# jackyko1991/vnet-tensorflow

Hardware: AMD Instinct MI355X
Metric: training patches/sec (128^3x1ch fp32) (higher is better)
Workload: dtype f32

## Files before the change

profiles/summarize.py:

```python
import csv
import json
import os
import shutil
import sys
from collections import defaultdict

LEGS = ("fp32", "x3", "c5", "c2")
KEEP = ("conv_kernel<", "wgrad_kernel<", "conv5_bf16", "wgrad5_bf16", "wgrad5_b16", "conv5_x3", "wgrad5_x3", "conv2_", "bn_", "input_")

FAMILIES = {
    "fp32": ("fp32", [("fwd", "conv_kernel<5, 1, 4, 8, 8, 4, 4, 1, false, 5, true", "2097152", 0),
                      ("bwd", "conv_kernel<5, 1, 4, 8, 8, 4, 4, 2, false, 5, false", "2097152", 0),
                      ("wgrad", "wgrad_kernel<5, 1, 4, 4, 16, 1, 16, 5", "131072", 0)]),
    "f32x3": ("x3", [("fwd", "conv5_x3_kernel<true, 1, false>", None, "longest"),
                     ("bwd", "conv5_x3_kernel<false, 2, false>", None, "longest"),
                     ("wgrad", "wgrad5_x3_kernel<false>", None, "longest")]),
    "bf16": ("c5", [("fwd", "conv5_bf16_c16pp_kernel<true>", None, "longest"),
                    ("bwd", "conv5_bf16_r32_kernel<false", None, 0),
                    ("wgrad", "wgrad5_bf16_rr_kernel<4, false>", None, 0)]),
}


def short(name):
    name = name.replace("(anonymous namespace)::", "").replace("void ", "")
    return name.split("(")[0]


def read_pass(path, counter):
    per_dispatch, meta = defaultdict(float), {}
    for r in csv.DictReader(open(path)):
        if r["Counter_Name"] != counter:
            continue
        key = int(r["Dispatch_Id"])
        per_dispatch[key] += float(r["Counter_Value"])
        meta[key] = (short(r["Kernel_Name"]), r["Grid_Size"], int(r["End_Timestamp"]) - int(r["Start_Timestamp"]))
    seqs = defaultdict(list)
    for key in sorted(per_dispatch):
        name, grid, dur = meta[key]
        seqs[(name, grid)].append((per_dispatch[key], dur))
    return seqs


def family_dispatches(src, here, tag):
    rows = []
    for fam, (leg, members) in FAMILIES.items():
        path = os.path.join(src, leg + "_kernel_trace.csv")
        if not os.path.exists(path):
            continue
        seqs, steps = defaultdict(list), 0
        trace = sorted(csv.DictReader(open(path)), key=lambda r: int(r["Start_Timestamp"]))
        for r in trace:
            name = short(r["Kernel_Name"])
            if name.startswith("softmax_dice_bwd_kernel"):
                steps += 1
            grid = r.get("Grid_Size") or str(int(r["Grid_Size_X"]) * int(r["Grid_Size_Y"]) * int(r["Grid_Size_Z"]))
            seqs[(name, grid)].append((int(r["Start_Timestamp"]), int(r["End_Timestamp"]) - int(r["Start_Timestamp"])))
        for role, pat, grid, pos in members:
            keys = [k for k in seqs if k[0].startswith(pat) and (grid is None or k[1] == grid)]
            if len(keys) != 1 or not steps:
                print("WARNING: %s/%s: %d kernels match" % (fam, role, len(keys)))
                continue
            seq = seqs[keys[0]]
            per_step = len(seq) // steps if len(seq) % steps == 0 else 1
            if pos == "longest":
                sel = [max(seq[i:i + per_step], key=lambda t: t[1]) for i in range(0, len(seq), per_step)]
            else:
                sel = seq[pos % per_step::per_step]
            for i, (t0, dur) in enumerate(sel):
                rows.append((fam, leg, role, keys[0][0], i, dur))
            d = sorted(t[1] for t in sel)
            print("%-6s %-6s %-40s n=%3d  avg %8.1f us  median %8.1f  min %8.1f  max %8.1f" %
                  (fam, role, keys[0][0][:40], len(d), sum(d) / len(d) / 1e3, d[len(d) // 2] / 1e3, d[0] / 1e3, d[-1] / 1e3))
    if rows:
        with open(os.path.join(here, tag + "_family_dispatches.csv"), "w") as f:
            f.write("family,leg,role,kernel,launch_index,duration_ns\n")
            for r in rows:
                f.write('%s,%s,%s,"%s",%d,%d\n' % r)


def main(src, tag):
    here = os.path.dirname(os.path.abspath(__file__))
    family_dispatches(src, here, tag)
    out = {"note": "per launch; KB from rocprofv3 --pmc (separate passes, one leg per run); fetch doubled per the gfx950 correction",
           "legs": {}, "families": {}}
    for leg in LEGS:
        st = os.path.join(src, leg + "_kernel_stats.csv")
        if os.path.exists(st):
            shutil.copy(st, os.path.join(here, "%s_kernel_stats_%s.csv" % (tag, leg)))
        seqs = {}
        for which, counter in (("fetch", "FETCH_SIZE"), ("write", "WRITE_SIZE")):
            path = os.path.join(src, "%s_%s_counter_collection.csv" % (leg, which))
            if os.path.exists(path):
                seqs[counter] = read_pass(path, counter)
        if not seqs:
            continue
        kern = {}
        for key in sorted(set().union(*[set(s) for s in seqs.values()])):
            name, grid = key
            if not name.startswith(KEEP):
# ... 63 lines not shown
```

vnet_tensorflow_amd/csrc/conv_kernels.h:

```cpp
#pragma once
#include "common.h"
#include <mutex>
#include <unordered_map>
#include <type_traits>
#include <vector>

namespace {

struct ConvArgs {
    const float* x0; const float* x1; int C0, C1, Cin;
    const float4* wp; const float* bias;
    float* y0; float* y1; int Cy0, Cy1, Cout;
    int B, Di, Hi, Wi, Do, Ho, Wo;
    int CQ;
    int CoutP;
    int nchunks, cps;
    int nbz, nby, nbx;
    int pad, padx;
    int vec_in, vec_out;
    float* part; size_t part_stride;
    int upO;
    int nz;
    int accum;
    const float* accsrc;
// ... 543 lines not shown
template <int KS, int STRIDE, int TZ, int TY, int TX, int NS, int TW, int KX = KS, bool IO16 = false>
__device__ __forceinline__ void wgrad_body(const WgradArgs& a, const int gid_x, const int gid_y, const int gid_z) {
#define VNET_WG_BID_X gid_x
#define VNET_WG_BID_Y gid_y
#define VNET_WG_BID_Z gid_z
#include "wgrad_body.inc"
#undef VNET_WG_BID_X
#undef VNET_WG_BID_Y
#undef VNET_WG_BID_Z
}

template <bool VEC>
__device__ __forceinline__ void wgrad_reduce_body(const float* __restrict__ part, int nsplit, int T3, int CinP, int CoutP,
                                                  int Cin, int Cout, float* __restrict__ dw, unsigned blk, unsigned nblk) {
    constexpr int W = VEC ? 4 : 1;
    __shared__ float sh[4][64 * W];
    const size_t total = (size_t)T3 * Cin * Cout / W;
    const size_t sstride = (size_t)T3 * CinP * CoutP;
    const int CoutG = Cout / W;
    const int o = threadIdx.x & 63, sg = threadIdx.x >> 6;
    for (size_t base = (size_t)blk * 64; base < total; base += (size_t)nblk * 64) {
        const size_t idx = base + o;
        float s[W];
#pragma unroll
        for (int j = 0; j < W; ++j) s[j] = 0.f;
        if (idx < total) {
            const int co = (int)(idx % CoutG) * W;
            const size_t r = idx / CoutG;
            const int ci = (int)(r % Cin), t = (int)(r / Cin);
            const float* p = part + ((size_t)t * CinP + ci) * CoutP + co;
            float acc[4][W];
#pragma unroll
            for (int u = 0; u < 4; ++u)
#pragma unroll
                for (int j = 0; j < W; ++j) acc[u][j] = 0.f;
            auto ld = [&](int k, float (&d)[W]) {
                if (VEC) { const float4 v = *reinterpret_cast<const float4*>(p + (size_t)k * sstride); d[0] += v.x; d[W > 1 ? 1 : 0] += v.y; d[W > 2 ? 2 : 0] += v.z; d[W > 3 ? 3 : 0] += v.w; }
                else d[0] += p[(size_t)k * sstride];
            };
            int k = sg;
            for (; k + 12 < nsplit; k += 16) { ld(k, acc[0]); ld(k + 4, acc[1]); ld(k + 8, acc[2]); ld(k + 12, acc[3]); }
            for (; k < nsplit; k += 4) ld(k, acc[0]);
#pragma unroll
            for (int j = 0; j < W; ++j) s[j] = (acc[0][j] + acc[1][j]) + (acc[2][j] + acc[3][j]);
        }
        __syncthreads();
#pragma unroll
        for (int j = 0; j < W; ++j) sh[sg][o * W + j] = s[j];
        __syncthreads();
        if (sg == 0 && idx < total) {
            float out[W];
#pragma unroll
            for (int j = 0; j < W; ++j) out[j] = sh[0][o * W + j] + sh[1][o * W + j] + sh[2][o * W + j] + sh[3][o * W + j];
            if (VEC) *reinterpret_cast<float4*>(dw + idx * 4) = make_float4(out[0], out[W > 1 ? 1 : 0], out[W > 2 ? 2 : 0], out[W > 3 ? 3 : 0]);
            else dw[idx] = out[0];
        }
    }
}

template <bool VEC>
__global__ void __launch_bounds__(256) wgrad_reduce_kernel(const float* __restrict__ part, int nsplit, int T3, int CinP, int CoutP,
                                                           int Cin, int Cout, float* __restrict__ dw) {
    wgrad_reduce_body<VEC>(part, nsplit, T3, CinP, CoutP, Cin, Cout, dw, blockIdx.x, gridDim.x);
}

}
namespace vnet_detail {
struct ReduceJob { const float* part; float* dw; int nsplit, T3, CinP, CoutP, Cin, Cout, vec; unsigned blk0; };
constexpr int REDUCE_BATCH = 32;
struct ReduceBatch { ReduceJob job[REDUCE_BATCH]; int n; };
struct DeferQueue { bool on = false; std::vector<ReduceJob> pending; };
struct DeferState { std::mutex mu; std::unordered_map<hipStream_t, DeferQueue> q; };
__attribute__((visibility("hidden"))) DeferState& defer_state();
struct Tuning {
    int wgrad_zs;
    int wgrad_rr;
    int conv_in4;
    double group_rounds;
    int group_debug;
    int bf16_deep;
    int bf16_deep_target;
    int bf16_c16pp;
    int x3_nb2;
    int f32_small;
};
__attribute__((visibility("hidden"))) Tuning& tuning();
}
namespace {
using vnet_detail::ReduceJob; using vnet_detail::ReduceBatch; using vnet_detail::REDUCE_BATCH;
using vnet_detail::DeferState; using vnet_detail::DeferQueue; using vnet_detail::defer_state; using vnet_detail::tuning;

__global__ void __launch_bounds__(256) wgrad_reduce_batched_kernel(ReduceBatch b) {
    int j = 0;
#pragma unroll 1
    for (int k = 1; k < b.n; ++k) if (blockIdx.x >= b.job[k].blk0) j = k;
    const ReduceJob& q = b.job[j];
    const unsigned nblk = (j + 1 < b.n ? b.job[j + 1].blk0 : gridDim.x) - q.blk0;
    if (q.vec) wgrad_reduce_body<true>(q.part, q.nsplit, q.T3, q.CinP, q.CoutP, q.Cin, q.Cout, q.dw, blockIdx.x - q.blk0, nblk);
    else wgrad_reduce_body<false>(q.part, q.nsplit, q.T3, q.CinP, q.CoutP, q.Cin, q.Cout, q.dw, blockIdx.x - q.blk0, nblk);
}


int launch_wgrad_reduce(const float* part, int nsplit, int T3, int CinP, int CoutP, int Cin, int Cout, float* dw, hipStream_t st) {
    const bool vec = (Cout % 4 == 0) && (CoutP % 4 == 0) && ((reinterpret_cast<uintptr_t>(dw) | reinterpret_cast<uintptr_t>(part)) & 15) == 0;
    {
        DeferState& ds = defer_state();
        std::lock_guard<std::mutex> lk(ds.mu);
        auto it = ds.q.find(st);
        if (it != ds.q.end() && it->second.on) {
            it->second.pending.push_back(ReduceJob{part, dw, nsplit, T3, CinP, CoutP, Cin, Cout, vec ? 1 : 0, 0u});
            return 0;
        }
    }
    const size_t total = (size_t)T3 * Cin * Cout / (vec ? 4 : 1);
    const int blocks = (int)min((size_t)4096, (total + 63) / 64);
    return with_bool(vec, [&](auto V) {
        return launch<wgrad_reduce_kernel<V>>(dim3(blocks), dim3(256), 0, st, part, nsplit, T3, CinP, CoutP, Cin, Cout, dw);
    });
}


__device__ __forceinline__ void pack_bf16_elem(int mode, const float* __restrict__ w, unsigned short* __restrict__ wp,
                                               int T, int I, int O, int ncob, size_t idx) {
    const int e = (int)(idx & 7);
    size_t q = idx >> 3;
    const int m = (int)(q & 31); q >>= 5;
    const int hf = (int)(q & 1); q >>= 1;
    const int cob = (int)(q % ncob); q /= ncob;
    const int t = (int)(q % T);
    const int chunk = (int)(q / T);
    const int k = chunk * 16 + hf * 8 + e, n = cob * 32 + m;
    float v = 0.f;
    if (mode == VNET_PACK_FWD_BF16) { if (k < I && n < O) v = w[((size_t)t * I + k) * O + n]; }
    else { if (k < O && n < I) v = w[((size_t)(T - 1 - t) * I + n) * O + k]; }
    wp[idx] = (unsigned short)(pk_bf16(v, 0.f) & 0xffffu);
}

#include "x3_pack.h"

__global__ void pack_kernel(int mode, const float* __restrict__ w, float* __restrict__ wp, int T, int I, int O,
                            int CQ, int NP, size_t total) {
    const bool r16 = (mode & VNET_PACK_ROUND_BF16) != 0;
    mode &= ~VNET_PACK_ROUND_BF16;
    for (size_t idx = (size_t)blockIdx.x * blockDim.x + threadIdx.x; idx < total; idx += (size_t)gridDim.x * blockDim.x) {
        const int r = (int)(idx & 3);
        size_t q = idx >> 2;
        const int n = (int)(q % NP); q /= NP;
        const int cq = (int)(q % CQ);
        const int t = (int)(q / CQ);
        const int k = cq * 4 + r;
        float v = 0.f;
        if (mode == VNET_PACK_FWD) {
            if (k < I && n < O) v = w[((size_t)t * I + k) * O + n];
        } else if (mode == VNET_PACK_BWD) {
            if (k < O && n < I) v = w[((size_t)(T - 1 - t) * I + n) * O + k];
        } else {
            if (k < I && n < 8 * O) v = w[(size_t)n * I + k];
        }
        wp[idx] = r16 ? bf_lo(pk_bf16(v, 0.f)) : v;
    }
}

#define VNET_PRIO_ALT(cond) do { if (cond) __builtin_amdgcn_s_setprio(1); else __builtin_amdgcn_s_setprio(0); } while (0)
#define VNET_PRIO_OFF() __builtin_amdgcn_s_setprio(0)

__global__ void __launch_bounds__(256) pack_batched_kernel(const long long* __restrict__ descs) {
// ... 1591 lines not shown
```

vnet_tensorflow_amd/csrc/conv_mfma.hip:

```cpp
#include "conv_kernels.h"
#include <string.h>

namespace vnet_detail {
DeferState& defer_state() { static DeferState s; return s; }
static Tuning tuning_from_env() {
    auto geti = [](const char* n, int d) { const char* e = getenv(n); return e ? atoi(e) : d; };
    Tuning t{};
    t.wgrad_zs = geti("VNET_WGRAD_ZS", 2); t.wgrad_rr = geti("VNET_WGRAD_RR", 1); t.conv_in4 = geti("VNET_CONV_IN4", 1);
    const char* g = getenv("VNET_WGRAD_GROUP_ROUNDS");
    t.group_rounds = g ? atof(g) : 2.0;
    t.group_debug = getenv("VNET_WGRAD_GROUP_DEBUG") ? 1 : 0;
    t.bf16_deep = geti("VNET_BF16_DEEP", 1); t.bf16_deep_target = geti("VNET_BF16_DEEP_TARGET", 256);
    t.f32_small = geti("VNET_F32_SMALL", 2); t.x3_nb2 = geti("VNET_X3_NB2", 1); t.bf16_c16pp = geti("VNET_BF16_C16PP", 1);
    return t;
}
Tuning& tuning() { static Tuning t = tuning_from_env(); return t; }
}

namespace {
double* option_slot(const char* name, int** ip) {
    vnet_detail::Tuning& t = vnet_detail::tuning();
    *ip = nullptr;
    if (!name) return nullptr;
    if (!strcmp(name, "WGRAD_ZS")) *ip = &t.wgrad_zs;
    else if (!strcmp(name, "WGRAD_RR")) *ip = &t.wgrad_rr;
    else if (!strcmp(name, "CONV_IN4")) *ip = &t.conv_in4;
    else if (!strcmp(name, "WGRAD_GROUP_DEBUG")) *ip = &t.group_debug;
    else if (!strcmp(name, "BF16_DEEP")) *ip = &t.bf16_deep;
    else if (!strcmp(name, "BF16_DEEP_TARGET")) *ip = &t.bf16_deep_target;
    else if (!strcmp(name, "F32_SMALL")) *ip = &t.f32_small;
    else if (!strcmp(name, "X3_NB2")) *ip = &t.x3_nb2;
    else if (!strcmp(name, "BF16_C16PP")) *ip = &t.bf16_c16pp;
    else if (!strcmp(name, "WGRAD_GROUP_ROUNDS")) return &t.group_rounds;
    return nullptr;
}
}

extern "C" {

double vnet_set_option(const char* name, double value) {
    int* ip; double* dp = option_slot(name, &ip);
    if (ip) { const double prev = *ip; *ip = (int)value; return prev; }
    if (dp) { const double prev = *dp; *dp = value; return prev; }
    return __builtin_nan("");
}
double vnet_get_option(const char* name) {
    int* ip; double* dp = option_slot(name, &ip);
    return ip ? (double)*ip : (dp ? *dp : __builtin_nan(""));
}

const char* vnet_version(void) { return "vnet_hip 0.2 (gfx950; fp32 MFMA 16x16x4, bf16 MFMA 32x32x16 / 16x16x32)"; }

size_t vnet_packed_weight_floats(int mode, int taps, int I, int O) {
    if (mode == VNET_PACK_FWD_X3 || mode == VNET_PACK_BWD_X3) {
        int nchunk, ncob; x3_packed_dims(mode == VNET_PACK_BWD_X3, I, O, &nchunk, &ncob);
        return (size_t)nchunk * X3_NPAIR * ncob * 3 * 256;
    }
    if (mode == VNET_PACK_FWD_BF16 || mode == VNET_PACK_BWD_BF16) {
        int nchunk, ncob; packed_dims_bf16(mode, I, O, &nchunk, &ncob);
        return (size_t)nchunk * taps * ncob * 512 / 2;
    }
    int Tp, CQ, NP; packed_dims(mode & ~VNET_PACK_ROUND_BF16, taps, I, O, &Tp, &CQ, &NP);
    return (size_t)Tp * CQ * NP * 4;
}

int vnet_pack_weights(int mode, const float* w, float* wp, int taps, int I, int O, void* stream) {
    if (!w || !wp || taps <= 0 || I <= 0 || O <= 0) return VNET_E_BADARG;
    if (mode == VNET_PACK_FWD_X3 || mode == VNET_PACK_BWD_X3) {
        if (taps != 125) return VNET_E_UNSUPPORTED;
        int nchunk, ncob; x3_packed_dims(mode == VNET_PACK_BWD_X3, I, O, &nchunk, &ncob);
        const uint32_t units = (uint32_t)nchunk * X3_NPAIR * ncob * 64;
        return launch<x3_pack_kernel>(dim3(min(4096u, (units + 255) / 256)), dim3(256), 0, (hipStream_t)stream,
                                      mode == VNET_PACK_BWD_X3 ? 1 : 0, w, reinterpret_cast<u32x4*>(wp), I, O, ncob, units);
    }
    if (mode == VNET_PACK_FWD_BF16 || mode == VNET_PACK_BWD_BF16) {
        int nchunk, ncob; packed_dims_bf16(mode, I, O, &nchunk, &ncob);
        const size_t total = (size_t)nchunk * taps * ncob * 512;
        const int blocks = (int)min((size_t)4096, (total + 255) / 256);
        return launch<pack_bf16_kernel>(dim3(blocks), dim3(256), 0, (hipStream_t)stream, mode, w,
                                        reinterpret_cast<unsigned short*>(wp), taps, I, O, ncob, total);
    }
    const int base = mode & ~VNET_PACK_ROUND_BF16;
    if (base < 0 || base > 2) return VNET_E_UNSUPPORTED;
    if (base == VNET_PACK_UP && taps != 8) return VNET_E_UNSUPPORTED;
    int Tp, CQ, NP; packed_dims(base, taps, I, O, &Tp, &CQ, &NP);
    const size_t total = (size_t)Tp * CQ * NP * 4;
    const int blocks = (int)min((size_t)4096, (total + 255) / 256);
    return launch<pack_kernel>(dim3(blocks), dim3(256), 0, (hipStream_t)stream, mode, w, wp, taps, I, O, CQ, NP, total);
}

int vnet_packed_dims(int mode, int taps, int I, int O, int* CQ, int* NP) {
    if (!CQ || !NP) return VNET_E_BADARG;
    if (mode == VNET_PACK_FWD_X3 || mode == VNET_PACK_BWD_X3) { x3_packed_dims(mode == VNET_PACK_BWD_X3, I, O, CQ, NP); return VNET_OK; }
    if (mode == VNET_PACK_FWD_BF16 || mode == VNET_PACK_BWD_BF16) { packed_dims_bf16(mode, I, O, CQ, NP); return VNET_OK; }
    mode &= ~VNET_PACK_ROUND_BF16;
    if (mode < 0 || mode > 2) return VNET_E_BADARG;
    int Tp; packed_dims(mode, taps, I, O, &Tp, CQ, NP);
    return VNET_OK;
}

int vnet_pack_weights_batched(const void* descs_dev, int n, void* stream) {
    if (!descs_dev || n <= 0) return VNET_E_BADARG;
    return launch<pack_batched_kernel>(dim3(512, n), dim3(256), 0, (hipStream_t)stream, (const long long*)descs_dev);
}

size_t vnet_conv_ws_bytes(int ks, int kx, int stride, int up, int Cin, int Cout, int B, int Do, int Ho, int Wo) {
    if (ks == 3 && (stride != 1 || up || (kx != 0 && kx != 3))) return 0;
    const int gridW = up ? (Wo + 1) / 2 : Wo;
    ConvPlan p = plan_conv(ks, stride, up, Cin, Cout, B, up ? (Do + 1) / 2 : Do, up ? (Ho + 1) / 2 : Ho, gridW, gridW);
    if (p.nsplit * p.nz <= 1) return 0;
    return (size_t)p.nsplit * p.nz * B * Do * Ho * Wo * round_up(Cout, 16) * sizeof(float);
}

int vnet_conv_stats_rows(int ks, int kx, int stride, int up, int Cin, int Cy0, int Cy1, int B, int Do, int Ho, int Wo) {
// ... 227 lines not shown
```

vnet_tensorflow_amd/csrc/conv_x3.h:

```cpp
#pragma once
#include "conv_kernels.h"

namespace {

constexpr int X3_TZ = 2, X3_TY = 8, X3_TX = 16;
constexpr int X3_IZ = X3_TZ + 4, X3_IY = X3_TY + 4, X3_IX = X3_TX + 4;
constexpr int X3_NV = X3_IZ * X3_IY * X3_IX;

template <bool W8>
struct X3G {
    static constexpr int TZ = W8 ? 4 : 2;
    static constexpr int IZ = TZ + 4, IY = X3_IY, IX = W8 ? 12 : X3_IX;
    static constexpr int ROWB = IX * 16;
    static constexpr int ZB = IY * ROWB + (W8 ? 64 : 0);
    static constexpr int PLANEB = IZ * ZB;
    static constexpr int PIECEB = 2 * PLANEB;
    static constexpr int TILEB = 3 * PIECEB;
    static constexpr int LDS = TILEB + 2 * 8 * 32 * 4;
    static constexpr int SPER = W8 ? 8 : 12;
};
static_assert(X3G<false>::PLANEB == X3_NV * 16 && X3G<false>::PLANEB % 256 == 0 && X3G<true>::PLANEB % 256 == 0, "tile planes");
static_assert((2 * X3G<true>::ZB) % 256 == 128, "lanes 8..15 of the narrow brick: the other half of the 256-byte bank row");
constexpr int X3_LDS = X3G<false>::LDS;

// ... 296 lines not shown
            const int oz = W8 ? bz * G::TZ + grp + 2 * (j >> 3) : bz * X3_TZ + grp, ox = W8 ? (j & 7) : bx * X3_TX + j;
            x3_for<2>([&](auto TI) {
                constexpr int t = decltype(TI)::value;
                const int oy = by * X3_TY + 2 * kw + t;
                if (oz < a.Do && oy < a.Ho && ox < a.Wo && co < a.Cout) {
                    const size_t ov = ((size_t)(b * a.Do + oz) * a.Ho + oy) * a.Wo + ox;
                    if (a.part) {
                        *reinterpret_cast<f32x4*>(a.part + (size_t)ks * a.part_stride + ov * a.CoutP + co) = o[t];
                        return;
                    }
                    float e[4] = {o[t][0] + bias4[0], o[t][1] + bias4[1], o[t][2] + bias4[2], o[t][3] + bias4[3]};
                    if constexpr (STATS) {
                        float4 rr = make_float4(0.f, 0.f, 0.f, 0.f);
                        if (a.res) rr = *reinterpret_cast<const float4*>(a.res + ov * a.Cout + co);
                        const float vv[4] = {e[0] + rr.x, e[1] + rr.y, e[2] + rr.z, e[3] + rr.w};
                        s1[0] += vv[0]; s1[1] += vv[1]; s1[2] += vv[2]; s1[3] += vv[3];
                        s2[0] += vv[0] * vv[0]; s2[1] += vv[1] * vv[1]; s2[2] += vv[2] * vv[2]; s2[3] += vv[3] * vv[3];
                    }
                    float* p = (co < a.Cy0) ? a.y0 + ov * a.Cy0 + co : a.y1 + ov * a.Cy1 + (co - a.Cy0);
                    if (a.accum) {
                        const float4 old = *reinterpret_cast<const float4*>(a.accsrc ? a.accsrc + ov * a.Cy0 + co : p);
                        e[0] += old.x; e[1] += old.y; e[2] += old.z; e[3] += old.w;
                    }
                    *reinterpret_cast<float4*>(p) = make_float4(e[0], e[1], e[2], e[3]);
                }
            });
            if constexpr (STATS) {
                x3_for<4>([&](auto KI) {
                    constexpr int k = decltype(KI)::value;
                    s1[k] = row16_sum(s1[k]); s2[k] = row16_sum(s2[k]);
                    if (j == 0) { sred[(nb * 8 + wave) * 32 + 4 * g + k] = s1[k]; sred[(nb * 8 + wave) * 32 + 16 + 4 * g + k] = s2[k]; }
                });
            }
            });
            __syncthreads();
            if constexpr (STATS) {
                int brick = (i_lo + slot + it * G8) / (ncobg * nks);
                x3_for<NB>([&](auto NBI) {
                    constexpr int nb = decltype(NBI)::value;
                    stats_row_write<8, 16>(sred + nb * 8 * 32, a.stats, (size_t)brick, (cob + nb) * 16, a.Cout, tid);
                });
            }
        }
        VNET_STAMP(6);
        if (last) zero_halo();
        if (more) tile_commit(((last ? 0 : lc + 1) & 1) ? 0x80000000u : 0u);
        VNET_STAMP(7);
        __syncthreads();
        VNET_STAMP(8);
        VNET_STAMP_FLUSH(step, wave, lane, 9);
    }
}

template <bool W8>
struct XWG {
    static constexpr int TZ = W8 ? 4 : 2;
    static constexpr int IZ = TZ + 4, IX = W8 ? 12 : X3_IX;
    static constexpr int XROW = IX * 32, XPLANE = X3_IY * XROW;
    static constexpr int XPB = IZ * XPLANE;
    static constexpr int DPB = 2 * X3_TY * 16 * 32;
    static constexpr int LDS = 3 * XPB + 3 * DPB;
    static constexpr int XHALF = W8 ? 2 * XPLANE : 8 * 32;
    static constexpr int XPER = W8 ? 8 : 12;
};
static_assert(XWG<false>::XROW % 256 == 128 && XWG<true>::XROW % 256 == 128, "row pairs of a k-step on disjoint banks");
constexpr int XW_LDS = XWG<false>::LDS;

__device__ __forceinline__ void xw_frag(bf16x8 (&F)[3], const unsigned char* lo, const unsigned char* hi, int pieceb) {
    typedef s16x4 __attribute__((address_space(3))) * lp;
#pragma unroll
    for (int s = 0; s < 3; ++s) {
        const s16x4 a = __builtin_amdgcn_ds_read_tr16_b64_v4i16((lp)(lo + s * pieceb));
        const s16x4 b = __builtin_amdgcn_ds_read_tr16_b64_v4i16((lp)(hi + s * pieceb));
        const s16x8 v = {a[0], a[1], a[2], a[3], b[0], b[1], b[2], b[3]};
        F[s] = __builtin_bit_cast(bf16x8, v);
    }
}

__device__ __forceinline__ void xw_mfma6(f32x4& acc, const bf16x8 (&A)[3], const bf16x8 (&B)[3]) {
#pragma unroll
    for (int k = 0; k < 6; ++k) acc = __builtin_amdgcn_mfma_f32_16x16x32_bf16(A[X3_PROD_A(k)], B[X3_PROD_B(k)], acc, 0, 0, 0);
}

template <bool W8>
__global__ void __launch_bounds__(512) __attribute__((amdgpu_waves_per_eu(2, 2))) wgrad5_x3_kernel(WgradArgs a) {
    constexpr int NT = 512;
    using G = XWG<W8>;
    constexpr int XW_XPB = G::XPB, XW_DPB = G::DPB, XW_XROW = G::XROW, XW_XPLANE = G::XPLANE;
    using XT = XTile<X3_IZ, X3_IY, X3_IX, NT>;
    static_assert(XT::PER == XWG<false>::XPER, "staging passes of the wide brick");
    extern __shared__ __attribute__((aligned(16))) unsigned char smem[];
    unsigned char* xt = smem;
    unsigned char* dyt = smem + 3 * XW_XPB;
    const int tid = threadIdx.x;
    const int lane = tid & 63, wave = __builtin_amdgcn_readfirstlane(tid >> 6);
    const int i = lane & 15, g = lane >> 4;
    const int split = blockIdx.x;
    const int chunk = blockIdx.y / a.ncob, cob = blockIdx.y - chunk * a.ncob;
    const int co0 = cob * 16;

    const int lane_x = W8 ? ((g & 1) * G::IX + (i >> 2)) * 32 + (g >> 1) * G::XHALF + (i & 3) * 8
                            : (((g & 1) * X3_IX + (g >> 1) * 8) + (i >> 2)) * 32 + (i & 3) * 8;
    const unsigned char* pb[3];
#pragma unroll
    for (int c = 0; c < 3; ++c) {
        const int q = 3 * wave + c, dz = q / 5, dx = q - dz * 5;
        pb[c] = xt + dz * XW_XPLANE + dx * 32 + lane_x;
    }
    const bool extra = wave < 5;
    const unsigned char* pe = xt + 4 * XW_XPLANE + (extra ? wave : 0) * XW_XROW + 4 * 32 + lane_x;
    const int lane_d = (((g & 1) * 16 + (g >> 1) * 8) + (i >> 2)) * 32 + (i & 3) * 8;
    const unsigned char* pa_lo = dyt + lane_d + (g & 1) * 128;
    const unsigned char* pa_hi = dyt + lane_d + (1 - (g & 1)) * 128;

    f32x4 acc[16];
#pragma unroll
    for (int t = 0; t < 16; ++t) acc[t] = f32x4{0.f, 0.f, 0.f, 0.f};

    float4 px[G::XPER], pd[2];
    auto brick_coords = [&](int brick, int& b, int& bz, int& by, int& bx) {
        bx = brick % a.nbx; brick /= a.nbx;
        by = brick % a.nby; brick /= a.nby;
        bz = brick % a.nbz; b = brick / a.nbz;
    };
    auto issue = [&](int brick) {
        int b, bz, by, bx;
        brick_coords(brick, b, bz, by, bx);
        if constexpr (W8) {
            const int stid = tid < 384 ? tid : tid - 128;
            const int iy = stid >> 5, col = stid & 31;
            const int c = chunk * 16 + (col & 3) * 4;
            const bool first = c < a.C0;
            const int cs = first ? a.C0 : a.C1;
            const float* src = (first ? a.x0 + c : a.x1 + (c - a.C0)) + (size_t)b * a.Di * a.Hi * a.Wi * cs;
            const int gz0 = bz * G::TZ - 2, gy = by * X3_TY - 2 + iy;
            const bool yok = (unsigned)gy < (unsigned)a.Hi;
            const int rs = a.Wi * cs, off0 = (gy * a.Wi + (col >> 2)) * cs;
#pragma unroll
            for (int k = 0; k < G::XPER; ++k) {
                const int gz = gz0 + k;
                const bool ok = yok && (unsigned)gz < (unsigned)a.Di;
                const float4 t = *reinterpret_cast<const float4*>(src + (ok ? off0 + gz * a.Hi * rs : 0));
                px[k] = ok ? t : make_float4(0.f, 0.f, 0.f, 0.f);
            }
        } else {
            XT::template issue_part<0, XT::PER>(px, a.x0, a.x1, a.C0, a.C1, chunk, b, bz * X3_TZ - 2, by * X3_TY - 2, bx * X3_TX - 2, a.Di, a.Hi, a.Wi, tid);
        }
#pragma unroll
        for (int k = 0; k < 2; ++k) {
            const int q = tid + k * NT;
            const int v = q >> 2, cq = q & 3;
            const int vx = v & 15, vy = (v >> 4) & 7, vz = v >> 7;
            const int oz = W8 ? bz * G::TZ + vz + 2 * (vx >> 3) : bz * X3_TZ + vz, oy = by * X3_TY + vy, ox = W8 ? (vx & 7) : bx * X3_TX + vx;
            const int c = co0 + cq * 4;
            const bool ok = oz < a.Do && oy < a.Ho && ox < a.Wo && c < a.Cout;
            const size_t ov = ok ? ((size_t)(b * a.Do + oz) * a.Ho + oy) * a.Wo + ox : 0;
            const float4 t = *reinterpret_cast<const float4*>(a.dy + ov * a.Cout + (ok ? c : 0));
            pd[k] = ok ? t : make_float4(0.f, 0.f, 0.f, 0.f);
        }
    };
    auto commit = [&](const bool neg) {
        if constexpr (W8) {
            const int stid = tid < 384 ? tid : tid - 128;
            unsigned char* base = xt + (stid >> 5) * XW_XROW + (((stid & 31) >> 2) + 2) * 32 + (stid & 3) * 8;
#pragma unroll
            for (int k = 0; k < G::XPER; ++k) {
                u32x2 h, m, l;
                x3_split4(px[k], h, m, l);
                unsigned char* dst = base + k * XW_XPLANE;
                *reinterpret_cast<u32x2*>(dst) = h;
                *reinterpret_cast<u32x2*>(dst + XW_XPB) = m;
                *reinterpret_cast<u32x2*>(dst + 2 * XW_XPB) = l;
            }
        } else {
        const int r0 = tid / XT::COLS, col = tid - r0 * XT::COLS;
        if (r0 < XT::RPI) {
            unsigned char* base = xt + (col >> 2) * 32 + (col & 3) * 8;
#pragma unroll
            for (int k = 0; k < XT::PER; ++k) {
                const int row = r0 + k * XT::RPI;
                u32x2 h, m, l;
                x3_split4(px[k], h, m, l);
                unsigned char* dst = base + row * XW_XROW;
                *reinterpret_cast<u32x2*>(dst) = h;
                *reinterpret_cast<u32x2*>(dst + XW_XPB) = m;
                *reinterpret_cast<u32x2*>(dst + 2 * XW_XPB) = l;
            }
        }
        }
#pragma unroll
        for (int k = 0; k < 2; ++k) {
            const int q = tid + k * NT;
            const int v = q >> 2, cq = q & 3;
            const int vx = v & 15, row = v >> 4;
            u32x2 h, m, l;
            const float4 dv = neg ? make_float4(-pd[k].x, -pd[k].y, -pd[k].z, -pd[k].w) : pd[k];
            x3_split4(dv, h, m, l);
            unsigned char* dst = dyt + (row * 16 + (vx ^ ((row & 1) << 2))) * 32 + cq * 8;
            *reinterpret_cast<u32x2*>(dst) = h;
            *reinterpret_cast<u32x2*>(dst + XW_DPB) = m;
            *reinterpret_cast<u32x2*>(dst + 2 * XW_DPB) = l;
        }
    };

    bool neg = false;
    if constexpr (W8) {
        for (int q = tid; q < 3 * G::IZ * X3_IY * 4 * 2; q += NT) {
            const int hf = q & 1, c = (q >> 1) & 3, row = (q >> 3) % (G::IZ * X3_IY), piece = q / (8 * G::IZ * X3_IY);
            *reinterpret_cast<u32x4*>(xt + piece * XW_XPB + row * XW_XROW + (c < 2 ? c : c + 8) * 32 + hf * 16) = u32x4{0u, 0u, 0u, 0u};
        }
    }
    if (split < a.nbrick) issue(split);
    for (int brick = split; brick < a.nbrick; brick += a.nsplit) {
        __syncthreads();
        commit(neg);
        __syncthreads();
        if (brick != split) {
#pragma unroll
            for (int t = 0; t < 16; ++t) acc[t] = -acc[t];
        }
        neg = !neg;
        auto plane = [&](const int zz) {
            if ((wave >> 2) ^ zz) __builtin_amdgcn_s_setprio(1); else __builtin_amdgcn_s_setprio(0);
            const int zx = zz * XW_XPLANE, zd = zz * (X3_TY * 16 * 32);
#pragma unroll
            for (int c = 0; c < 3; ++c) {
                const unsigned char* p = pb[c] + zx;
                bf16x8 F[5][3], A[3], An[3];
#pragma unroll
                for (int r = 0; r < 5; ++r) xw_frag(F[r], p + r * XW_XROW, p + r * XW_XROW + 128, XW_XPB);
                xw_frag(An, pa_lo + zd, pa_hi + zd, XW_DPB);
#pragma unroll
                for (int s = 0; s < 4; ++s) {
#pragma unroll
                    for (int q = 0; q < 3; ++q) A[q] = An[q];
                    if (s + 1 < 4) xw_frag(An, pa_lo + zd + (s + 1) * 1024, pa_hi + zd + (s + 1) * 1024, XW_DPB);
                    __builtin_amdgcn_sched_barrier(0);
                    xw_mfma6(acc[c * 5 + 0], A, F[(2 * s + 0) % 5]);
                    xw_mfma6(acc[c * 5 + 1], A, F[(2 * s + 1) % 5]);
                    __builtin_amdgcn_sched_barrier(0);
                    if (s + 1 < 4) {
                        xw_frag(F[(2 * s + 0) % 5], p + (2 * s + 5) * XW_XROW, p + (2 * s + 5) * XW_XROW + 128, XW_XPB);
                        xw_frag(F[(2 * s + 1) % 5], p + (2 * s + 6) * XW_XROW, p + (2 * s + 6) * XW_XROW + 128, XW_XPB);
                    }
                    __builtin_amdgcn_sched_barrier(0);
                    xw_mfma6(acc[c * 5 + 2], A, F[(2 * s + 2) % 5]);
                    xw_mfma6(acc[c * 5 + 3], A, F[(2 * s + 3) % 5]);
                    xw_mfma6(acc[c * 5 + 4], A, F[(2 * s + 4) % 5]);
                    __builtin_amdgcn_sched_barrier(0);
                }
            }
            if (extra) {
                const unsigned char* p = pe + zx;
                bf16x8 E[3], En[3], A[3], An[3];
                xw_frag(En, p, p + 128, XW_XPB);
                xw_frag(An, pa_lo + zd, pa_hi + zd, XW_DPB);
#pragma unroll
                for (int s = 0; s < 4; ++s) {
#pragma unroll
                    for (int q = 0; q < 3; ++q) { A[q] = An[q]; E[q] = En[q]; }
                    if (s + 1 < 4) {
                        xw_frag(An, pa_lo + zd + (s + 1) * 1024, pa_hi + zd + (s + 1) * 1024, XW_DPB);
                        xw_frag(En, p + (2 * s + 2) * XW_XROW, p + (2 * s + 2) * XW_XROW + 128, XW_XPB);
                    }
                    __builtin_amdgcn_sched_barrier(0);
                    xw_mfma6(acc[15], A, E);
                    __builtin_amdgcn_sched_barrier(0);
                }
            }
        };
        plane(0);
        __builtin_amdgcn_sched_barrier(0);
        issue(brick + a.nsplit < a.nbrick ? brick + a.nsplit : brick);
        __builtin_amdgcn_sched_barrier(0);
        plane(1);
    }
    __builtin_amdgcn_s_setprio(0);
    if (!neg) {
#pragma unroll
        for (int t = 0; t < 16; ++t) acc[t] = -acc[t];
    }
#pragma unroll
    for (int t = 0; t < 16; ++t) {
        int tap;
        if (t < 15) { const int q = 3 * wave + t / 5, dz = q / 5, dx = q - dz * 5; tap = (dz * 5 + t % 5) * 5 + dx; }
        else { if (!extra) continue; tap = (4 * 5 + wave) * 5 + 4; }
        float* dst = a.part + ((size_t)(split * 125 + tap) * a.CinP + chunk * 16 + i) * a.CoutP + co0 + g * 4;
        const f32x4 r = acc[t];
        *reinterpret_cast<float4*>(dst) = make_float4(r.x, r.y, r.z, r.w);
    }
}

inline int x3_conv_nbz(int D, int W) { return W == 8 ? ceil_div(D, X3G<true>::TZ) : ceil_div(D, X3_TZ); }
inline int x3_conv_bricks(int B, int D, int H, int W) { return B * x3_conv_nbz(D, W) * ceil_div(H, X3_TY) * ceil_div(W, X3_TX); }
struct X3WgradPlan { int nbz, nby, nbx, nbrick, nsplit, nblk; };
inline X3WgradPlan x3_plan_wgrad(int Cin, int Cout, int B, int D, int H, int W) {
    X3WgradPlan p{};
    p.nbz = x3_conv_nbz(D, W); p.nby = ceil_div(H, X3_TY); p.nbx = ceil_div(W, X3_TX);
    p.nbrick = B * p.nbz * p.nby * p.nbx;
    p.nblk = (Cin / 16) * (Cout / 16);
    p.nsplit = max(1, min(p.nbrick, ceil_div(256, p.nblk)));
    return p;
}
inline bool x3_wgrad_ok(int C0, int C1, int Cout, int B, int D, int H, int W) {
    if (C0 <= 0 || Cout <= 0 || (C0 & 15) || (C1 & 15) || (Cout & 15) || (W < 16 && W != 8)) return false;
    const X3WgradPlan p = x3_plan_wgrad(C0 + C1, Cout, B, D, H, W);
    return p.nbrick >= (W == 8 ? 2 : 4) * p.nsplit;
}

struct X3Plan { int ok, nks, cps; long items; };
inline X3Plan x3_plan_conv(int C0, int C1, int Cy0, int Cy1, int B, int D, int H, int W) {
    X3Plan p{0, 1, 0, 0};
    if (C0 <= 0 || Cy0 <= 0 || (C0 & 15) || (C1 & 15) || (Cy0 & 15) || (Cy1 & 15) || (W < 16 && W != 8)) return p;
    const int nch = (C0 + C1) / 16;
    p.items = (long)x3_conv_bricks(B, D, H, W) * ((Cy0 + Cy1) / 16);
    p.cps = nch;
    while (p.items * p.nks < 256 && p.cps % 2 == 0 && p.cps >= 4) { p.nks *= 2; p.cps /= 2; }
    p.ok = p.items * p.nks >= 192;
    return p;
}
inline bool x3_conv_ok(int C0, int C1, int Cy0, int Cy1, int B, int D, int H, int W) { return x3_plan_conv(C0, C1, Cy0, Cy1, B, D, H, W).ok != 0; }

}
```

vnet_tensorflow_amd/csrc/conv_x3.hip:

```cpp
#include "conv_x3.h"

namespace {

int x3_grid() { return device_cus() / 8 * 8; }

}

extern "C" {

int vnet_conv_x3_ok(int C0, int C1, int Cy0, int Cy1, int B, int D, int H, int W) {
    return x3_conv_ok(C0, C1, Cy0, Cy1, B, D, H, W) ? 1 : 0;
}

int vnet_conv_x3_stats_rows(int Cin, int Cout, int B, int D, int H, int W) {
    if (Cin <= 0 || Cout <= 0 || B <= 0 || D <= 0 || H <= 0 || W <= 0) return 0;
    const X3Plan p = x3_plan_conv(Cin, 0, Cout, 0, B, D, H, W);
    if (p.nks > 1) {
        if (Cout > 256 || 256 % Cout) return 0;
        const size_t total = (size_t)B * D * H * W * Cout;
        return (int)min((size_t)2048, (total + 255) / 256);
    }
    return x3_conv_bricks(B, D, H, W);
}

size_t vnet_conv_x3_ws_bytes(int Cin, int Cout, int B, int D, int H, int W) {
    if (Cin <= 0 || Cout <= 0 || (Cin & 15) || (Cout & 15) || B <= 0 || D <= 0 || H <= 0 || W <= 0) return 0;
    const X3Plan p = x3_plan_conv(Cin, 0, Cout, 0, B, D, H, W);
    return p.nks > 1 ? (size_t)p.nks * B * D * H * W * Cout * sizeof(float) : 0;
}

int vnet_conv_fwd_x3(const float* x0, int C0, const float* x1, int C1, const void* wp, const float* bias,
                     float* y0, int Cy0, float* y1, int Cy1, int B, int D, int H, int W,
                     const float* acc, const float* res, float* stats, void* ws, size_t ws_bytes, void* stream) {
    if (!x0 || !wp || !y0 || C0 <= 0 || Cy0 <= 0 || B <= 0 || D <= 0 || H <= 0 || W <= 0) return VNET_E_BADARG;
    if ((C1 > 0 && !x1) || (Cy1 > 0 && !y1) || C1 < 0 || Cy1 < 0) return VNET_E_BADARG;
    if ((C0 & 15) || (C1 & 15) || (Cy0 & 15) || (Cy1 & 15)) return VNET_E_UNSUPPORTED;
    if ((stats || res) && Cy1 > 0) return VNET_E_BADARG;
    if (acc && acc != y0 && Cy1 > 0) return VNET_E_BADARG;
    if ((long long)D * H * W * (C0 > C1 ? C0 : C1) >= (1ll << 31)) return VNET_E_UNSUPPORTED;
    ConvArgs a{};
    a.x0 = x0; a.x1 = x1; a.C0 = C0; a.C1 = C1; a.Cin = C0 + C1;
    a.wp = reinterpret_cast<const float4*>(wp); a.bias = bias;
    a.y0 = y0; a.y1 = y1; a.Cy0 = Cy0; a.Cy1 = Cy1; a.Cout = Cy0 + Cy1;
    a.B = B; a.Di = D; a.Hi = H; a.Wi = W; a.Do = D; a.Ho = H; a.Wo = W;
    a.nchunks = a.Cin / 16; a.CQ = a.nchunks * 4; a.CoutP = a.Cout;
    a.nbz = x3_conv_nbz(D, W); a.nby = ceil_div(H, X3_TY); a.nbx = ceil_div(W, X3_TX);
    a.pad = 2; a.padx = 2; a.vec_in = 1; a.vec_out = 1;
    a.accum = acc ? 1 : 0; a.accsrc = (acc && acc != y0) ? acc : nullptr;
    a.res = res; a.stats = stats;
    const X3Plan p = x3_plan_conv(a.Cin, 0, a.Cout, 0, B, D, H, W);
    a.nz = p.nks; a.cps = p.cps ? p.cps : a.nchunks;
    const size_t nvox = (size_t)B * D * H * W;
    if (p.nks > 1) {
        const size_t need = (size_t)p.nks * nvox * a.Cout * sizeof(float);
        if (!ws || ws_bytes < need) return VNET_E_WORKSPACE;
        if (stats && (a.Cout > 256 || 256 % a.Cout)) return VNET_E_UNSUPPORTED;
        a.part = reinterpret_cast<float*>(ws); a.part_stride = nvox * a.Cout;
    }
    hipStream_t st = (hipStream_t)stream;
    const int grid = x3_grid();
    const bool w8 = W == 8;
    const bool nb2 = !w8 && (a.Cout % 32 == 0) && p.items * p.nks >= 2 * (long)grid && tuning().x3_nb2 != 0;
    const int e = with_bool(stats && p.nks == 1, [&](auto S) {
        return w8 ? launch<conv5_x3_kernel<S, 1, true>>(dim3(grid), dim3(512), X3G<true>::LDS, st, a)
                  : with_int<2, 1>(nb2 ? 2 : 1, [&](auto NB) {
                        return launch<conv5_x3_kernel<S, NB, false>>(dim3(grid), dim3(512), X3G<false>::LDS, st, a);
                    });
    });
    if (e || p.nks <= 1) return e;
    const size_t total = nvox * a.Cout;
    const int blocks = (int)min((size_t)2048, (total + 255) / 256);
    return launch<splitk_reduce_kernel>(dim3(blocks), dim3(256), 0, st, a.part, a.part_stride, p.nks, bias,
                                        y0, y1, Cy0, Cy1, a.CoutP, nvox, a.accum, a.res, a.stats, a.accsrc);
}

int vnet_wgrad_x3_ok(int C0, int C1, int Cout, int B, int D, int H, int W) {
    return x3_wgrad_ok(C0, C1, Cout, B, D, H, W) ? 1 : 0;
}

size_t vnet_wgrad_x3_ws_bytes(int Cin, int Cout, int B, int D, int H, int W) {
    if (Cin <= 0 || Cout <= 0 || (Cin & 15) || (Cout & 15) || B <= 0 || D <= 0 || H <= 0 || W <= 0) return 0;
    const X3WgradPlan p = x3_plan_wgrad(Cin, Cout, B, D, H, W);
    return (size_t)p.nsplit * 125 * Cin * Cout * sizeof(float);
}

int vnet_conv_wgrad_x3(const float* x0, int C0, const float* x1, int C1, const float* dy, int Cout, float* dw,
                       int B, int D, int H, int W, void* ws, size_t ws_bytes, void* stream) {
    if (!x0 || !dy || !dw || C0 <= 0 || Cout <= 0 || B <= 0 || C1 < 0 || (C1 > 0 && !x1)) return VNET_E_BADARG;
    if (D <= 0 || H <= 0 || W <= 0) return VNET_E_BADARG;
    if ((C0 & 15) || (C1 & 15) || (Cout & 15)) return VNET_E_UNSUPPORTED;
    if ((long long)D * H * W * (C0 > C1 ? C0 : C1) >= (1ll << 31)) return VNET_E_UNSUPPORTED;
    hipStream_t st = (hipStream_t)stream;
    WgradArgs a{};
    a.x0 = x0; a.x1 = x1; a.C0 = C0; a.C1 = C1; a.Cin = C0 + C1; a.dy = dy; a.Cout = Cout;
    a.B = B; a.Di = D; a.Hi = H; a.Wi = W; a.Do = D; a.Ho = H; a.Wo = W;
    a.CinP = a.Cin; a.CoutP = Cout; a.pad = 2; a.padx = 2; a.vec_in = 1; a.vec_dy = 1;
    const X3WgradPlan p = x3_plan_wgrad(a.Cin, Cout, B, D, H, W);
    a.ncob = Cout / 16; a.nbz = p.nbz; a.nby = p.nby; a.nbx = p.nbx; a.nbrick = p.nbrick; a.nsplit = p.nsplit;
    const size_t need = (size_t)p.nsplit * 125 * a.Cin * Cout * sizeof(float);
    const bool direct = p.nsplit == 1;
    if (!direct && (!ws || ws_bytes < need)) return VNET_E_WORKSPACE;
    a.part = direct ? dw : reinterpret_cast<float*>(ws);
    const int e = with_bool(W == 8, [&](auto N) { return launch<wgrad5_x3_kernel<N>>(dim3(p.nsplit, p.nblk), dim3(512), XWG<N>::LDS, st, a); });
    if (e || direct) return e;
    return launch_wgrad_reduce(a.part, p.nsplit, 125, a.CinP, a.CoutP, a.Cin, Cout, dw, st);
}

#ifdef VNET_STAMPS
int vnet_debug_set_stamps_x3(void* buf) { return (int)hipMemcpyToSymbol(HIP_SYMBOL(g_stamps), &buf, sizeof(buf)); }
#endif

}
```

Before: 67.25.

## Reuse input planes across z-adjacent bricks in x3 wgrad via a ring buffer

The wide-brick wgrad5_x3 kernel now walks bricks in z-major order, with each split taking a contiguous run of bricks. The input tile is kept in a six-plane LDS ring, so moving to the next z brick loads and commits only one new plane pair instead of restaging the whole halo tile. This cuts global loads and LDS staging of the input. The cost is extra fill work at column starts, changed brick-to-split assignment for all paths (including the 8^3 path), and more complex slot indexing. It is enabled by default via VNET_X3_WGRAD_ZRING.

```diff
diff --git a/profiles/summarize.py b/profiles/summarize.py
--- a/profiles/summarize.py
+++ b/profiles/summarize.py
@@ -14,7 +14,7 @@
                       ("wgrad", "wgrad_kernel<5, 1, 4, 4, 16, 1, 16, 5", "131072", 0)]),
     "f32x3": ("x3", [("fwd", "conv5_x3_kernel<true, 1, false>", None, "longest"),
                      ("bwd", "conv5_x3_kernel<false, 2, false>", None, "longest"),
-                     ("wgrad", "wgrad5_x3_kernel<false>", None, "longest")]),
+                     ("wgrad", "wgrad5_x3_kernel<false", None, "longest")]),
     "bf16": ("c5", [("fwd", "conv5_bf16_c16pp_kernel<true>", None, "longest"),
                     ("bwd", "conv5_bf16_r32_kernel<false", None, 0),
                     ("wgrad", "wgrad5_bf16_rr_kernel<4, false>", None, 0)]),
diff --git a/vnet_tensorflow_amd/csrc/conv_kernels.h b/vnet_tensorflow_amd/csrc/conv_kernels.h
--- a/vnet_tensorflow_amd/csrc/conv_kernels.h
+++ b/vnet_tensorflow_amd/csrc/conv_kernels.h
@@ -649,6 +649,7 @@
     int bf16_deep_target;
     int bf16_c16pp;
     int x3_nb2;
+    int x3_wgrad_zring;
     int f32_small;
 };
 __attribute__((visibility("hidden"))) Tuning& tuning();
diff --git a/vnet_tensorflow_amd/csrc/conv_mfma.hip b/vnet_tensorflow_amd/csrc/conv_mfma.hip
--- a/vnet_tensorflow_amd/csrc/conv_mfma.hip
+++ b/vnet_tensorflow_amd/csrc/conv_mfma.hip
@@ -12,6 +12,7 @@
     t.group_debug = getenv("VNET_WGRAD_GROUP_DEBUG") ? 1 : 0;
     t.bf16_deep = geti("VNET_BF16_DEEP", 1); t.bf16_deep_target = geti("VNET_BF16_DEEP_TARGET", 256);
     t.f32_small = geti("VNET_F32_SMALL", 2); t.x3_nb2 = geti("VNET_X3_NB2", 1); t.bf16_c16pp = geti("VNET_BF16_C16PP", 1);
+    t.x3_wgrad_zring = geti("VNET_X3_WGRAD_ZRING", 1);
     return t;
 }
 Tuning& tuning() { static Tuning t = tuning_from_env(); return t; }
@@ -30,6 +31,7 @@
     else if (!strcmp(name, "BF16_DEEP_TARGET")) *ip = &t.bf16_deep_target;
     else if (!strcmp(name, "F32_SMALL")) *ip = &t.f32_small;
     else if (!strcmp(name, "X3_NB2")) *ip = &t.x3_nb2;
+    else if (!strcmp(name, "X3_WGRAD_ZRING")) *ip = &t.x3_wgrad_zring;
     else if (!strcmp(name, "BF16_C16PP")) *ip = &t.bf16_c16pp;
     else if (!strcmp(name, "WGRAD_GROUP_ROUNDS")) return &t.group_rounds;
     return nullptr;
diff --git a/vnet_tensorflow_amd/csrc/conv_x3.h b/vnet_tensorflow_amd/csrc/conv_x3.h
--- a/vnet_tensorflow_amd/csrc/conv_x3.h
+++ b/vnet_tensorflow_amd/csrc/conv_x3.h
@@ -402,13 +402,17 @@
     for (int k = 0; k < 6; ++k) acc = __builtin_amdgcn_mfma_f32_16x16x32_bf16(A[X3_PROD_A(k)], B[X3_PROD_B(k)], acc, 0, 0, 0);
 }
 
-template <bool W8>
+template <bool W8, bool RING = false>
 __global__ void __launch_bounds__(512) __attribute__((amdgpu_waves_per_eu(2, 2))) wgrad5_x3_kernel(WgradArgs a) {
+    static_assert(!(W8 && RING), "the narrow brick (two bricks per column at 8^3) keeps whole-tile staging");
     constexpr int NT = 512;
     using G = XWG<W8>;
     constexpr int XW_XPB = G::XPB, XW_DPB = G::DPB, XW_XROW = G::XROW, XW_XPLANE = G::XPLANE;
     using XT = XTile<X3_IZ, X3_IY, X3_IX, NT>;
+    using XT2 = XTile<2, X3_IY, X3_IX, NT>;
     static_assert(XT::PER == XWG<false>::XPER, "staging passes of the wide brick");
+    static_assert(XT2::PER == 4 && XT2::RPI == XT::RPI && XT2::PER * XT2::RPI == 2 * X3_IY, "a plane pair is four whole staging passes");
+    constexpr int NPX = RING ? XT2::PER : G::XPER;
     extern __shared__ __attribute__((aligned(16))) unsigned char smem[];
     unsigned char* xt = smem;
     unsigned char* dyt = smem + 3 * XW_XPB;
@@ -422,13 +426,15 @@
     const int lane_x = W8 ? ((g & 1) * G::IX + (i >> 2)) * 32 + (g >> 1) * G::XHALF + (i & 3) * 8
                             : (((g & 1) * X3_IX + (g >> 1) * 8) + (i >> 2)) * 32 + (i & 3) * 8;
     const unsigned char* pb[3];
+    int pdz[3];
 #pragma unroll
     for (int c = 0; c < 3; ++c) {
         const int q = 3 * wave + c, dz = q / 5, dx = q - dz * 5;
-        pb[c] = xt + dz * XW_XPLANE + dx * 32 + lane_x;
+        pdz[c] = dz;
+        pb[c] = xt + dx * 32 + lane_x;
     }
     const bool extra = wave < 5;
-    const unsigned char* pe = xt + 4 * XW_XPLANE + (extra ? wave : 0) * XW_XROW + 4 * 32 + lane_x;
+    const unsigned char* pe = xt + (extra ? wave : 0) * XW_XROW + 4 * 32 + lane_x;
     const int lane_d = (((g & 1) * 16 + (g >> 1) * 8) + (i >> 2)) * 32 + (i & 3) * 8;
     const unsigned char* pa_lo = dyt + lane_d + (g & 1) * 128;
     const unsigned char* pa_hi = dyt + lane_d + (1 - (g & 1)) * 128;
@@ -437,13 +443,13 @@
 #pragma unroll
     for (int t = 0; t < 16; ++t) acc[t] = f32x4{0.f, 0.f, 0.f, 0.f};
 
-    float4 px[G::XPER], pd[2];
+    float4 px[NPX], pd[2];
     auto brick_coords = [&](int brick, int& b, int& bz, int& by, int& bx) {
+        bz = brick % a.nbz; brick /= a.nbz;
         bx = brick % a.nbx; brick /= a.nbx;
-        by = brick % a.nby; brick /= a.nby;
-        bz = brick % a.nbz; b = brick / a.nbz;
-    };
-    auto issue = [&](int brick) {
+        by = brick % a.nby; b = brick / a.nby;
+    };
+    auto issue_x = [&](int brick, int pp) {
         int b, bz, by, bx;
         brick_coords(brick, b, bz, by, bx);
         if constexpr (W8) {
@@ -463,9 +469,15 @@
                 const float4 t = *reinterpret_cast<const float4*>(src + (ok ? off0 + gz * a.Hi * rs : 0));
                 px[k] = ok ? t : make_float4(0.f, 0.f, 0.f, 0.f);
             }
+        } else if constexpr (RING) {
+            XT2::template issue_part<0, XT2::PER>(px, a.x0, a.x1, a.C0, a.C1, chunk, b, bz * X3_TZ - 2 + 2 * pp, by * X3_TY - 2, bx * X3_TX - 2, a.Di, a.Hi, a.Wi, tid);
         } else {
             XT::template issue_part<0, XT::PER>(px, a.x0, a.x1, a.C0, a.C1, chunk, b, bz * X3_TZ - 2, by * X3_TY - 2, bx * X3_TX - 2, a.Di, a.Hi, a.Wi, tid);
         }
+    };
+    auto issue_dy = [&](int brick) {
+        int b, bz, by, bx;
+        brick_coords(brick, b, bz, by, bx);
 #pragma unroll
         for (int k = 0; k < 2; ++k) {
             const int q = tid + k * NT;
@@ -479,7 +491,7 @@
             pd[k] = ok ? t : make_float4(0.f, 0.f, 0.f, 0.f);
         }
     };
-    auto commit = [&](const bool neg) {
+    auto commit_x = [&](const int pairoff) {
         if constexpr (W8) {
             const int stid = tid < 384 ? tid : tid - 128;
             unsigned char* base = xt + (stid >> 5) * XW_XROW + (((stid & 31) >> 2) + 2) * 32 + (stid & 3) * 8;
@@ -495,9 +507,9 @@
         } else {
         const int r0 = tid / XT::COLS, col = tid - r0 * XT::COLS;
         if (r0 < XT::RPI) {
-            unsigned char* base = xt + (col >> 2) * 32 + (col & 3) * 8;
-#pragma unroll
-            for (int k = 0; k < XT::PER; ++k) {
+            unsigned char* base = xt + pairoff + (col >> 2) * 32 + (col & 3) * 8;
+#pragma unroll
+            for (int k = 0; k < NPX; ++k) {
                 const int row = r0 + k * XT::RPI;
                 u32x2 h, m, l;
                 x3_split4(px[k], h, m, l);
@@ -508,6 +520,8 @@
             }
         }
         }
+    };
+    auto commit_dy = [&](const bool neg) {
 #pragma unroll
         for (int k = 0; k < 2; ++k) {
             const int q = tid + k * NT;
@@ -530,22 +544,40 @@
             *reinterpret_cast<u32x4*>(xt + piece * XW_XPB + row * XW_XROW + (c < 2 ? c : c + 8) * 32 + hf * 16) = u32x4{0u, 0u, 0u, 0u};
         }
     }
-    if (split < a.nbrick) issue(split);
-    for (int brick = split; brick < a.nbrick; brick += a.nsplit) {
+    const int run = (a.nbrick + a.nsplit - 1) / a.nsplit;
+    const int lo = split * run, hi = min(a.nbrick, lo + run);
+    if (lo < hi) { issue_x(lo, 0); issue_dy(lo); }
+    bool fill = true;
+    for (int brick = lo; brick < hi; ++brick) {
+        const int bz = brick % a.nbz;
+        const int ring = RING ? 2 * (bz % 3) : 0;
         __syncthreads();
-        commit(neg);
+        if constexpr (RING) {
+            commit_x((fill ? ring : (ring + 4) % 6) * XW_XPLANE);
+            commit_dy(neg);
+            if (fill) {
+                issue_x(brick, 1);
+                commit_x(((ring + 2) % 6) * XW_XPLANE);
+                issue_x(brick, 2);
+                commit_x(((ring + 4) % 6) * XW_XPLANE);
+            }
+        } else {
+            commit_x(0);
+            commit_dy(neg);
+        }
         __syncthreads();
-        if (brick != split) {
+        if (brick != lo) {
 #pragma unroll
             for (int t = 0; t < 16; ++t) acc[t] = -acc[t];
         }
         neg = !neg;
         auto plane = [&](const int zz) {
             if ((wave >> 2) ^ zz) __builtin_amdgcn_s_setprio(1); else __builtin_amdgcn_s_setprio(0);
-            const int zx = zz * XW_XPLANE, zd = zz * (X3_TY * 16 * 32);
+            const int zd = zz * (X3_TY * 16 * 32);
+            auto slot = [&](int dz) { const int t = ring + dz + zz; return (t >= 6 ? t - 6 : t) * XW_XPLANE; };
 #pragma unroll
             for (int c = 0; c < 3; ++c) {
-                const unsigned char* p = pb[c] + zx;
+                const unsigned char* p = pb[c] + slot(pdz[c]);
                 bf16x8 F[5][3], A[3], An[3];
 #pragma unroll
                 for (int r = 0; r < 5; ++r) xw_frag(F[r], p + r * XW_XROW, p + r * XW_XROW + 128, XW_XPB);
@@ -571,7 +603,7 @@
                 }
             }
             if (extra) {
-                const unsigned char* p = pe + zx;
+                const unsigned char* p = pe + slot(4);
                 bf16x8 E[3], En[3], A[3], An[3];
                 xw_frag(En, p, p + 128, XW_XPB);
                 xw_frag(An, pa_lo + zd, pa_hi + zd, XW_DPB);
@@ -591,7 +623,12 @@
         };
         plane(0);
         __builtin_amdgcn_sched_barrier(0);
-        issue(brick + a.nsplit < a.nbrick ? brick + a.nsplit : brick);
+        {
+            const int next = brick + 1 < hi ? brick + 1 : brick;
+            fill = bz + 1 == a.nbz;
+            issue_x(next, fill ? 0 : 2);
+            issue_dy(next);
+        }
         __builtin_amdgcn_sched_barrier(0);
         plane(1);
     }
diff --git a/vnet_tensorflow_amd/csrc/conv_x3.hip b/vnet_tensorflow_amd/csrc/conv_x3.hip
--- a/vnet_tensorflow_amd/csrc/conv_x3.hip
+++ b/vnet_tensorflow_amd/csrc/conv_x3.hip
@@ -101,7 +101,10 @@
     const bool direct = p.nsplit == 1;
     if (!direct && (!ws || ws_bytes < need)) return VNET_E_WORKSPACE;
     a.part = direct ? dw : reinterpret_cast<float*>(ws);
-    const int e = with_bool(W == 8, [&](auto N) { return launch<wgrad5_x3_kernel<N>>(dim3(p.nsplit, p.nblk), dim3(512), XWG<N>::LDS, st, a); });
+    const int e = W == 8 ? launch<wgrad5_x3_kernel<true>>(dim3(p.nsplit, p.nblk), dim3(512), XWG<true>::LDS, st, a)
+                         : with_bool(tuning().x3_wgrad_zring != 0, [&](auto R) {
+                               return launch<wgrad5_x3_kernel<false, R>>(dim3(p.nsplit, p.nblk), dim3(512), XWG<false>::LDS, st, a);
+                           });
     if (e || direct) return e;
     return launch_wgrad_reduce(a.part, p.nsplit, 125, a.CinP, a.CoutP, a.Cin, Cout, dw, st);
 }
```

After: 67.81, median of 6. No clear change (+0.8%).
